# takah29/2d-fluid-simulator

Measured on AMD Instinct MI355X. Metric: simulation steps/sec + Poisson-sweep HBM GB/s (% roofline), res 4096², 1/2/4/8 GPU, higher is better.
Workload: dtype f32; 1 GPU; bc=5 res=4096 (8192x4096 cells) scheme=cip vc=5.0 RB-SOR(1.3, 2 iters) Re=1e+06 dt=0.05/res; BASELINE.json configs[2]; cells=33554432, fluid_cells=22424499, parallelism=y-slab x1

## Files before the change

### 2d-fluid-simulator_amd/csrc/fs_core.hip

```cpp
#include <algorithm>
#include <cstdio>
#include <cstdlib>
#include <cstring>
#include <cxxabi.h>
#include <mutex>
#include <numeric>
#include <type_traits>
#include <unordered_map>

#include "fs_launch.h"
#include "fs_tracer.h"

namespace fs {

static thread_local std::string g_err;
void set_error(const std::string &msg) { g_err = msg; }
int hip_fail(hipError_t e, const char *what, const char *file, int line)
{
    char buf[512];
    snprintf(buf, sizeof buf, "HIP error %d (%s) in %s at %s:%d", (int)e, hipGetErrorString(e), what, file, line);
    g_err = buf;
    return FS_ERR_HIP;
}

// ... 83 lines not shown
        c->prof_ms[r.name_id] += ms;
        c->prof_pool.push_back(r.start);
        c->prof_pool.push_back(r.stop);
    }
    c->prof_recs.clear();
    return FS_OK;
}

const fs_ctx::TileList *tile_list(fs_ctx *c, int lanes, int rt, bool stacked, int group, int nbx, int nby, int cls, int reach, int wgw, int jb, int je, int parent_rt)
{
    if (c->h_act4.empty() || nbx > 0xfff || nby > 0xffff || lanes > 4 || c->rows > 0xffff) return nullptr;
    if (je < 0) je = c->rows;
    if (parent_rt == rt) parent_rt = 0;
    if (parent_rt && (wgw != 1 || parent_rt % rt != 0 || parent_rt > 64)) return nullptr;
    if (cls == 3 && !(rt == 8 && parent_rt == 16 && wgw == 1 && lanes == 2)) return nullptr;
    const fs_ctx::TileKey key{{lanes, rt, stacked ? 1 : 0, group, cls, reach, wgw, parent_rt, jb, je}};
    auto it = c->tile_lists.find(key);
    if (it != c->tile_lists.end()) return it->second.d ? &it->second : nullptr;
    if (c->capturing || c->tape_rec || c->tile_lists.size() >= 512) { ++c->tile_list_misses; return nullptr; }
    const std::vector<uint8_t> &act = lanes == 4 ? c->h_act4 : (lanes == 2 ? c->h_act2 : c->h_act2w);
    const int ow = geo_owners(lanes), waves = (c->X / geo_cells(lanes) + ow - 1) / ow, Y = c->rows;
    std::vector<uint32_t> per[8];
    bool any_hint = false;
    auto plain_box = [&](int wx0, int wx1, int p0, int p1) -> bool {
        if (wx0 <= 0 || wx1 >= waves || p0 - reach < 0 || p1 + reach > Y) return false;
        for (int wx = wx0; wx < wx1; ++wx)
            for (int j = p0 - reach; j < p1 + reach; ++j)
                if (act[(size_t)wx * Y + j] & 2) return false;
        return true;
    };
    const int groups = (nby + group - 1) / group;
    constexpr bool col_major = true;
    for (int xcd = 0; xcd < 8; ++xcd)
        for (int lg = 0; lg * 8 + xcd < groups; ++lg)
            for (int o = 0; o < group * nbx; ++o) {
                const int ly = col_major ? o % group : o / nbx, bx = col_major ? o / group : o % nbx;
                const int by = (lg * 8 + xcd) * group + ly;
                if (by >= nby) continue;
                {
                    const int wx0 = stacked ? bx : bx * wgw, wx1 = std::min(waves, stacked ? bx + 1 : bx * wgw + wgw);
                    const int j0 = jb + (stacked ? by * wgw : by) * rt, j1 = std::min(je, jb + (stacked ? by * wgw + wgw : by + 1) * rt);
                    bool any = false;
                    for (int wx = wx0; wx < wx1 && !any; ++wx)
                        for (int j = j0; j < j1; ++j)
                            if (act[(size_t)wx * Y + j] & 1) { any = true; break; }
                    if (cls == 3) {
                        const int p0 = jb + (j0 - jb) / parent_rt * parent_rt, p1 = std::min(je, p0 + parent_rt);
                        if (p1 - p0 == parent_rt && plain_box(wx0, wx1, p0, p1)) {
                            if (j0 == p0) per[xcd].push_back((1u << 28) | ((uint32_t)by << 12) | (uint32_t)bx);
                        } else if (any) {
                            uint32_t h = 0u;
                            for (int s = 0; s < 2; ++s)
                                for (int j = j0 + 4 * s; j < std::min(j1, j0 + 4 * s + 4); ++j)
                                    if (act[(size_t)bx * Y + j] & 4) { h |= 2u << s; break; }
                            per[xcd].push_back((h << 28) | ((uint32_t)by << 12) | (uint32_t)bx);
                        }
                        any_hint = true;
                        continue;
                    }
                    if (any && cls) {
                        int p0 = j0, p1 = j1, full_rows = (stacked ? wgw : 1) * rt;
                        if (parent_rt) { p0 = jb + (j0 - jb) / parent_rt * parent_rt; p1 = std::min(je, p0 + parent_rt); full_rows = parent_rt; }
                        any = (p1 - p0 == full_rows && plain_box(wx0, wx1, p0, p1)) == (cls == 1);
                    }
                    uint32_t hints = 0u;
// ... 3 lines not shown
                            const int t0 = jb + (stacked ? by * wgw + w : by) * rt, t1 = std::min(je, t0 + rt);
                            if (wx >= waves || t0 >= je) continue;
                            const bool plain = plain_box(wx, wx + 1, t0, t1);
                            if (plain) hints |= 1u << w;
                        }
                        any_hint = any_hint || hints != 0u;
                    }
                    if (any && cls == 2 && wgw == 1) {
                        for (int j = j0; j < j1; ++j)
                            if (act[(size_t)bx * Y + j] & 4) { hints |= 2u; break; }
                    }
                    if (any) per[xcd].push_back((hints << 28) | ((uint32_t)by << 12) | (uint32_t)bx);
                }
            }
    if ((!cls || cls == 3) && any_hint && wgw == 1) {
        for (auto &v : per) std::stable_partition(v.begin(), v.end(), [](uint32_t e) { return ((e >> 28) & 1u) == 0u; });
    }
    size_t K = 0, total = 0;
    for (auto &v : per) total += v.size();
    if (total >= 64) {
        const size_t target = (total + 7) / 8;
        for (int d = 0; d < 8; ++d)
            while (per[d].size() > target) {
                int r = 0;
                for (int x = 1; x < 8; ++x) if (per[x].size() < per[r].size()) r = x;
                if (per[r].size() >= target) break;
                const size_t n = std::min(per[d].size() - target, target - per[r].size());
                per[r].insert(per[r].end(), per[d].end() - n, per[d].end());
                per[d].resize(per[d].size() - n);
            }
    }
    for (auto &v : per) K = std::max(K, v.size());
    fs_ctx::TileList tl;
    if (K > 0 && (cls || any_hint || total < (size_t)nbx * nby)) {
        std::vector<uint32_t> h(K * 8, 0xffffffffu);
        for (int xcd = 0; xcd < 8; ++xcd)
            for (size_t k = 0; k < per[xcd].size(); ++k) h[k * 8 + xcd] = per[xcd][k];
        if (hipMalloc(&tl.d, h.size() * sizeof(uint32_t)) == hipSuccess &&
            hipMemcpyAsync(tl.d, h.data(), h.size() * sizeof(uint32_t), hipMemcpyHostToDevice, c->stream) == hipSuccess &&
            hipStreamSynchronize(c->stream) == hipSuccess)
            { tl.per_xcd = (int)K; tl.count = (int)total; }
        else { if (tl.d) hipFree(tl.d); tl.d = nullptr; }
    }
    auto &slot = c->tile_lists[key] = tl;
    return slot.d ? &slot : nullptr;
}

static void tile_lists_free(fs_ctx *c)
{
    for (auto &kv : c->tile_lists) if (kv.second.d) hipFree(kv.second.d);
    c->tile_lists.clear();
}

int check_rows(const fs_ctx *c, int jb, int je)
{
    if (!(0 <= jb && jb <= je && je <= c->rows)) {
// ... 345 lines not shown
        int bv = 0, bd = 0;
        e = hipGetDeviceProperties(&prop, device);
        if (e == hipSuccess) e = dtype == 0 ? hipOccupancyMaxActiveBlocksPerMultiprocessor(&bv, k_velocity_bc_limit<float>, 256, 0)
                                            : hipOccupancyMaxActiveBlocksPerMultiprocessor(&bv, k_velocity_bc_limit<double>, 256, 0);
        if (e == hipSuccess) e = dtype == 0 ? hipOccupancyMaxActiveBlocksPerMultiprocessor(&bd, k_dye_bc_limit<float>, 256, 0)
                                            : hipOccupancyMaxActiveBlocksPerMultiprocessor(&bd, k_dye_bc_limit<double>, 256, 0);
        if (e == hipSuccess) c->barrier_wgs = std::min(bv, bd) * prop.multiProcessorCount / 2;
    }
    c->nwx = (nx / 4 + 61) / 62;
    if (e != hipSuccess) { fs_destroy(c); return hip_fail(e, "hipMalloc(ctx)", __FILE__, __LINE__); }
    if (const char *s = getenv("FS_MARCH")) c->use_march = atoi(s) != 0;
    if (const char *s = getenv("FS_TILE_LIST")) c->tile_list_mask = atoi(s);
    if (const char *s = getenv("FS_LIMIT_GATE")) c->limit_gate = atoi(s) != 0;
    if (const char *s = getenv("FS_FUSE_K2")) c->fuse_k2 = std::max(0, std::min(2, atoi(s)));
    if (const char *s = getenv("FS_RBPAIR_SPLIT")) c->rbpair_split = atoi(s);
    if (const char *s = getenv("FS_SMALL_CELLS")) c->small_cells = (size_t)atoll(s);
    c->stack_mask = XCD_RBSOR | XCD_ADVECT | XCD_GRAD;
    c->use_pairs = c->use_march && nx % 2 == 0;
    if (nx % 4 != 0) c->use_march = false;
    *out = c;
    return FS_OK;
}

int fs_destroy(fs_ctx *ctx)
{
    if (!ctx) return FS_OK;
    hipSetDevice(ctx->device);
    if (ctx->stream) hipStreamSynchronize(ctx->stream);
    fs_comm_destroy(ctx);
    for (auto g : ctx->graphs) if (g) hipGraphExecDestroy(g);
// ... 111 lines not shown
    tile_lists_free(ctx);
    ctx->h_act4.clear(); ctx->h_act2.clear(); ctx->h_act2w.clear();
    if (ctx->X % 2 == 0 && ctx->tile_list_mask && ctx->rows <= 0xffff) {
        const int X = ctx->X, Y = ctx->Y, R = ctx->rows, g0 = ctx->y0 - ctx->halo;
        struct Geo { std::vector<uint8_t> *act; int w, halo; } geos[3] = {{&ctx->h_act4, 248, 4}, {&ctx->h_act2, 120, 4}, {&ctx->h_act2w, 124, 2}};
        for (const Geo &ge : geos) {
            const int w = ge.w, n = (X + w - 1) / w;
            ge.act->assign((size_t)n * R, 0);
            for (int i = 0; i < X; ++i) {
                const uint8_t *m = mask_xy + (size_t)i * Y, *b = ctx->h_bcmap.data() + (size_t)i * Y;
                uint8_t *a = ge.act->data() + (size_t)(i / w) * R;
                const int r = i % w;
                uint8_t *h = r < ge.halo && i / w > 0 ? a - R : (r >= w - ge.halo && i / w + 1 < n ? a + R : nullptr);
                for (int lr = 0; lr < R; ++lr) {
                    const int j = g0 + lr;
                    if (j < 0 || j >= Y) { a[lr] |= 2; if (h) h[lr] |= 2; continue; }
                    const uint8_t nf = m[j] != 0 ? 2 : 4;
                    a[lr] |= (uint8_t)((m[j] != 1) | (b[j] != 0)) | nf;
                    if (h) h[lr] |= nf;
                }
            }
        }
    }
    std::vector<uint8_t>().swap(ctx->h_bcmap);
    if (rc) return rc;
    if (ctx->X % 4 == 0) {
        FS_KLAUNCH(k_lazy_flags, dim3((ctx->nwx * ctx->rows + 3) / 4), dim3(256), 0, ctx->stream, ctx->grid(), ctx->nwx, ctx->d_bcmap, ctx->d_lazyflags);
        FS_HIP(hipGetLastError());
        const size_t cap = (size_t)ctx->nwx * ctx->rows;
        if (!ctx->d_pairlist) FS_HIP(hipMalloc(&ctx->d_pairlist, (2 * cap + 2) * sizeof(uint32_t)));
        unsigned *d_count = (unsigned *)(ctx->d_pairlist + 2 * cap);
        FS_HIP(hipMemsetAsync(d_count, 0, 2 * sizeof(unsigned), ctx->stream));
// ... 1275 lines not shown
```

### 2d-fluid-simulator_amd/csrc/fs_host.h

```cpp
#pragma once
#include <hip/hip_runtime.h>
#include <stdint.h>

#include <array>
#include <cmath>
#include <functional>
#include <map>
#include <set>
#include <string>
#include <vector>

#include "../../include/fs_hip.h"
#include "fs_device.h"
#include "fs_kernels.h"
#include "fs_march.h"
#include "fs_rbpair.h"
#include "fs_jquad.h"
#include "fs_k34n.h"
#include "fs_history.h"

namespace fs {

void set_error(const std::string &msg);
int hip_fail(hipError_t e, const char *what, const char *file, int line);
// ... 44 lines not shown

struct fs_ctx {
    int device = 0;
    int X = 0, Y = 0, dtype = 0, y0 = 0, nyl = 0, halo = 0;
    int rows = 0, P = 0, Pm = 0;
    size_t esize = 4;
    hipStream_t stream = nullptr;
    uint8_t *d_mask = nullptr;
    uint8_t *d_bcmap = nullptr;
    uint8_t *d_lazyflags = nullptr;
    std::vector<uint8_t> h_bcmap;
    bool lazy_ok = false;
    bool rb_pair_ok = false;
    bool jq_ok = false;
    int rbpair_split = 1;
    size_t small_cells = (size_t)1 << 21;
    uint32_t *d_pairlist = nullptr; int n_pairlist[2] = {0, 0};
    int nwx = 0;
    void *d_bc_const = nullptr, *d_bc_dye = nullptr;
    bool mask_set = false, bc_incomplete = false;
    int bc_radius_vel = 0, bc_radius_prs = 0;
    fs::BcOpsDev ops_vel, ops_prs, ops_dye;
    void *d_stage = nullptr;
    size_t stage_bytes = 0;
    double *d_acc = nullptr;
    int barrier_wgs = 0;
    unsigned *d_sync = nullptr;
    double *d_partial = nullptr;
    size_t partial_cap = 0;
    double *d_stats = nullptr;
// ... 19 lines not shown
    std::set<fs_history *> histories;
    std::vector<fs_history *> deferred_hist;
    std::set<fs_mean *> means;
    std::vector<fs_mean *> deferred_mean;
    std::set<fs_tracer *> tracers;
    std::vector<fs_tracer *> deferred_tracer;
    std::vector<void *> deferred_accum;
    bool use_march = true;
    bool use_pairs = true;
    int fuse_k2 = 2;
    bool limit_gate = true;
    int stack_mask = 0;

    int tile_list_mask = 1 | 2 | 4 | 8 | 32;
    std::vector<uint8_t> h_act4, h_act2, h_act2w;
    struct TileList { uint32_t *d = nullptr; int per_xcd = 0; int count = 0; };
    using TileKey = std::array<int, 10>;
    std::map<TileKey, TileList> tile_lists;

    fs::Grid grid() const
    {
        fs::Grid g;
        g.tiles = nullptr;
        g.X = X; g.P = P; g.Pm = Pm; g.rows = rows;
        int jlo = halo - y0, jhi = halo - y0 + (Y - 1);
        g.jlo = jlo < 0 ? 0 : jlo;
        g.jhi = jhi > rows - 1 ? rows - 1 : jhi;
        g.ybase = y0 - halo;
        g.mask = d_mask;
        return g;
    }
};
// ... 109 lines not shown
```

### 2d-fluid-simulator_amd/csrc/fs_pressure.hip

```cpp
#include "fs_launch.h"
#include "fs_stats.h"
#include "fs_mean.h"

static_assert(fs::STATS_N == FS_FLOW_NSTAT, "fs_stats.h and include/fs_hip.h disagree on the slots");
static_assert(fs::MEAN_PLANES == FS_MEAN_NPLANE, "fs_mean.h and include/fs_hip.h disagree on the planes");

namespace fs {
void history_release(fs_history *h)
{
    if (h->d_probes) hipFree(h->d_probes);
    if (h->d_faces) hipFree(h->d_faces);
    if (h->d_ring) hipFree(h->d_ring);
    if (h->d_state) hipFree(h->d_state);
    if (h->d_partial) hipFree(h->d_partial);
    delete h;
}
void mean_release(fs_mean *m)
{
    if (m->d_sums) hipFree(m->d_sums);
    if (m->d_state) hipFree(m->d_state);
    delete m;
}
}

// ... 186 lines not shown
    FS_REQUIRE(pc_out != pc && pc_out != pn && pn != pc, "the finishing pass needs three distinct pressure fields");
    FS_ROWS();
    if (!(ctx->jq_ok && ctx->use_march && ctx->dtype == 0)) { set_error("this mask / precision does not admit the multi-sweep Jacobi passes (fs_jacobi_quad_ok)"); return FS_ERR_UNSUPPORTED; }
    using T = float;
    const OvGrid og = ov_grid_lanes(ctx, row_begin, row_end, 4, 1, XCD_RBSOR, 2, true, 0, 2);
    return launch(ctx, "jacobi_finish", [=] {
        FS_KLAUNCH((k_jacobi_finish<2, 4, T>), og.grid, dim3(og.threads), 0, ctx->stream, og.g, og.nbx, og.nby, row_begin, row_end,
                           (const uint8_t *)ctx->d_bcmap, (T *)pc_out->d, (T *)pn->d, (const T *)pc->d, (const T *)src->d);
    });
}

int fs_rbsor_pair_ok(const fs_ctx *ctx, int *ok)
{
    FS_REQUIRE(ctx && ok, "null argument");
    *ok = ctx->mask_set && ctx->rb_pair_ok && ctx->use_pairs ? 1 : 0;
    return FS_OK;
}

int fs_rbsor_pair(fs_ctx *ctx, double dt, double dx, double omega, fs_field *pc_out, fs_field *pn_out, const fs_field *pc, const fs_field *pn,
                  const fs_field *vc, int full, int row_begin, int row_end)
{
    FS_REQUIRE(ctx, "ctx is null");
    FS_FIELD(pc_out, 1); FS_FIELD(pn_out, 1); FS_FIELD(pc, 1); FS_FIELD(pn, 1); FS_FIELD(vc, 2);
    FS_REQUIRE(pc_out != pn_out && pc_out != pc && pc_out != pn && pn_out != pc && pn_out != pn && pc != pn, "the two-iteration pass needs four distinct pressure fields");
    FS_ROWS();
    if (!(ctx->rb_pair_ok && ctx->use_pairs)) {
        set_error("this mask does not admit the two-iteration red-black pass (fs_rbsor_pair_ok)");
        return FS_ERR_UNSUPPORTED;
    }
    const Grid gg = ctx->grid();
// ... 402 lines not shown
```

### 2d-fluid-simulator_amd/csrc/fs_rbpair.h

```cpp
#pragma once
#include "fs_march.h"

namespace fs {

#ifndef FS_RBP_MIRROR
#define FS_RBP_MIRROR 1
#endif

template <typename T, int N> struct LV { T a[N]; };
template <typename T, int N> struct LVec;
template <> struct LVec<float, 4> { using type = float4; };
template <> struct LVec<float, 2> { using type = float2; };
template <> struct LVec<double, 2> { using type = double2; };
template <int N> struct LMaskWord;
template <> struct LMaskWord<4> { using type = uint32_t; };
template <> struct LMaskWord<2> { using type = uint16_t; };

template <typename T, int N>
__device__ __forceinline__ LV<T, N> lv_load(const T *row, int i0)
{
    const typename LVec<T, N>::type q = load_row_quad<typename LVec<T, N>::type, T>(row, i0);
    LV<T, N> r;
    if constexpr (N == 4) { r.a[0] = q.x; r.a[1] = q.y; r.a[2] = q.z; r.a[3] = q.w; }
    else { r.a[0] = q.x; r.a[1] = q.y; }
// ... 165 lines not shown

template <typename T, int N>
__device__ __forceinline__ LV<T, N> lv_bc_row(const LaneMapN<N> &lm, const LV<T, N> &m, const LV<T, N> &c, const LV<T, N> &n, uint32_t code)
{
    if (!__any(lv_sel_target<N>(code) != 0u)) return c;
    const T cl = lv_left<T, N>(lm, c), cr = lv_right<T, N>(lm, c);
    LV<T, N> o;
#pragma unroll
    for (int q = 0; q < N; ++q) {
        const T sL = q == 0 ? cl : c.a[q == 0 ? 0 : q - 1], sR = q == N - 1 ? cr : c.a[q == N - 1 ? q : q + 1];
        o.a[q] = lazy_value((code >> (8 * q)) & 0xffu, c.a[q], sL, sR, m.a[q], n.a[q]);
    }
    return o;
}

template <int PAR, int COLOR, typename T, int N>
__device__ __forceinline__ void rbp_relax(const Konst<T> &k, const LaneMapN<N> &lm, unsigned fluid, const LV<T, N> &m, const LV<T, N> &ctr, const LV<T, N> &p,
                                          const LV<T, N> &s2, const LV<T, N> &s3, LV<T, N> &out)
{
    const T pl = lv_left<T, N>(lm, ctr), pr = lv_right<T, N>(lm, ctr);
#pragma unroll
    for (int c = 0; c < N; ++c) {
        if (((c + PAR) & 1) != COLOR) continue;
        const T pE = c == N - 1 ? pr : ctr.a[c == N - 1 ? c : c + 1], pW = c == 0 ? pl : ctr.a[c == 0 ? 0 : c - 1];
        const T pred = predict_from(pE, pW, p.a[c], m.a[c], s2.a[c], s3.a[c]);
        const T val = k.om1 * ctr.a[c] + k.om * pred;
        out.a[c] = (fluid & (1u << c)) ? val : out.a[c];
    }
}

template <int N, int RT, int PAR0, int DM, bool BND, bool FULL, typename T, bool MIRROR = false>
__device__ __forceinline__ void rbsor_pair_tile(const Grid &g, const Konst<T> &k, const LaneMapN<N> &lm_in, int i0, int j0, int je, const unsigned (&fl)[RT + 8],
                                                const uint8_t *bcmap, T *C, T *D, const T *A, const T *B, const T *v)
{
    static_assert(!(MIRROR && (BND || FULL)), "only plain tiles are mirrored");
    constexpr int W = RT + 8;
    constexpr int UP = MIRROR ? -1 : 1;
    constexpr int PARW = MIRROR ? PAR0 + 1 : PAR0;
#define FS_ROW(w) (MIRROR ? j0 + RT + 3 - (w) : j0 - 4 + (w))
    using R = LV<T, N>;
    constexpr unsigned ALL = (1u << N) - 1u;
    const LaneMapN<N> lm = BND ? lm_in : LaneMapN<N>{lm_in.i0, lm_in.owner, false, false};
// ... 55 lines not shown
    }
#pragma unroll
    for (int w = 4; w <= W - 5; ++w) {
        const int j = FS_ROW(w);
        if (j >= je) continue;
        const unsigned sel = FULL ? ALL : (FS_FL(w) | (BND ? lv_sel_target<N>(code[w]) : 0u));
        if (lm.owner && sel) {
            lv_store_sel<T, N>(C + idx<1, T>(g, 0, i0, j), P4[w], sel);
            lv_store_sel<T, N>(D + idx<1, T>(g, 0, i0, j), VB[w], sel);
        }
    }
#undef FS_FL
#undef FS_ROW
}

template <int N, int RT, int PAR0, int DM, bool MIRROR, typename T>
__device__ __forceinline__ void rbsor_pair_stack_tile(const Grid &g, const Konst<T> &k, const LaneMapN<N> &lm_in, int i0, int j0,
                                                      T *C, T *D, const T *A, const T *B, const T *v, typename LVec<T, N>::type (*xch)[2][64], int slot)
{
    constexpr int W = RT + 5;
    constexpr int UP = MIRROR ? -1 : 1;
    constexpr int PARW = MIRROR ? PAR0 + 1 : PAR0;
#define FS_ROW(w) (MIRROR ? j0 + RT + 3 - (w) : j0 - 4 + (w))
    using R = LV<T, N>;
    using Q = typename LVec<T, N>::type;
    constexpr unsigned ALL = (1u << N) - 1u;
    const LaneMapN<N> lm{lm_in.i0, lm_in.owner, false, false};
    const int lane = threadIdx.x & 63;
    R PA[W], VX[W], VY[W], PB[W];
#pragma unroll
    for (int w = 0; w < W; ++w) {
        const int j = clampy(g, FS_ROW(w));
        PA[w] = lv_field<1, T, N>(A, g, 0, i0, j);
// ... 3 lines not shown
    }
    R S2[W], S3[W];
#pragma unroll
    for (int w = 1; w <= W - 2; ++w) {
        const T xl = lv_left<T, N>(lm, VX[w]), xr = lv_right<T, N>(lm, VX[w]);
        const T yl = lv_left<T, N>(lm, VY[w]), yr = lv_right<T, N>(lm, VY[w]);
#pragma unroll
        for (int c = 0; c < N; ++c) {
            const T xE = c == N - 1 ? xr : VX[w].a[c == N - 1 ? c : c + 1], xW = c == 0 ? xl : VX[w].a[c == 0 ? 0 : c - 1];
            const T yE = c == N - 1 ? yr : VY[w].a[c == N - 1 ? c : c + 1], yW = c == 0 ? yl : VY[w].a[c == 0 ? 0 : c - 1];
            source_from<DM>(k, xE, xW, yE, yW, VX[w + UP].a[c], VX[w - UP].a[c], VY[w + UP].a[c], VY[w - UP].a[c], S2[w].a[c], S3[w].a[c]);
        }
    }
    auto put = [&](int e, const R &r) { Q q; q.x = r.a[0]; q.y = r.a[1]; xch[e][slot][lane] = q; };
    auto get = [&](int e) { const Q q = xch[e][1 - slot][lane]; R r; r.a[0] = q.x; r.a[1] = q.y; return r; };
#pragma unroll
    for (int w = 1; w <= W - 2; ++w) {
        if ((PARW + w) & 1) rbp_relax<1, 1>(k, lm, ALL, PA[w - UP], PA[w], PA[w + UP], S2[w], S3[w], PB[w]);
        else                rbp_relax<0, 1>(k, lm, ALL, PA[w - UP], PA[w], PA[w + UP], S2[w], S3[w], PB[w]);
    }
    put(0, PB[W - 2]);
    __syncthreads();
    PB[W - 1] = get(0);
    R P2[W];
#pragma unroll
    for (int w = 2; w <= W - 2; ++w) {
        P2[w] = PB[w];
        if ((PARW + w) & 1) rbp_relax<1, 0>(k, lm, ALL, PB[w - UP], PB[w], PB[w + UP], S2[w], S3[w], P2[w]);
        else                rbp_relax<0, 0>(k, lm, ALL, PB[w - UP], PB[w], PB[w + UP], S2[w], S3[w], P2[w]);
    }
    put(1, P2[W - 2]);
    __syncthreads();
    P2[W - 1] = get(1);
    R P3[W];
#pragma unroll
    for (int w = 3; w <= W - 2; ++w) {
        P3[w] = PA[w];
        if ((PARW + w) & 1) rbp_relax<1, 1>(k, lm, ALL, P2[w - UP], P2[w], P2[w + UP], S2[w], S3[w], P3[w]);
        else                rbp_relax<0, 1>(k, lm, ALL, P2[w - UP], P2[w], P2[w + UP], S2[w], S3[w], P3[w]);
    }
    put(2, P3[W - 2]);
    __syncthreads();
    P3[W - 1] = get(2);
    R P4[W];
#pragma unroll
    for (int w = 4; w <= W - 2; ++w) {
        P4[w] = P3[w];
        if ((PARW + w) & 1) rbp_relax<1, 0>(k, lm, ALL, P3[w - UP], P3[w], P3[w + UP], S2[w], S3[w], P4[w]);
        else                rbp_relax<0, 0>(k, lm, ALL, P3[w - UP], P3[w], P3[w + UP], S2[w], S3[w], P4[w]);
    }
    if (lm.owner) {
#pragma unroll
        for (int w = 4; w <= W - 2; ++w) {
            lv_store_row<1, T, N>(C, g, 0, i0, FS_ROW(w), P4[w]);
            lv_store_row<1, T, N>(D, g, 0, i0, FS_ROW(w), P2[w]);
        }
    }
#undef FS_ROW
}

template <int N, int RT, int PAR0, int DM, int PATH, bool FULL, typename T>
__device__ __forceinline__ void rbsor_pair_wave_at(const Grid &g, const Konst<T> &k, int wx, int ty, bool hint, bool bnd_fluid, int jb, int je,
                                                   const uint8_t *bcmap, T *C, T *D, const T *A, const T *B, const T *v)
{
    constexpr int W = RT + 8;
    const LaneMapN<N> lm = lane_map_n<N>(g, wx);
// ... 42 lines not shown

template <int N, int PAR0, int DM, typename T>
__global__ __launch_bounds__(128) void k_rbsor_pair_all(Grid g, Konst<T> k, int nbx, int nby, int jb, int je, const uint8_t *bcmap, T *C, T *D, const T *A, const T *B, const T *v)
{
    constexpr int RT = 8;
    __shared__ typename LVec<T, N>::type xch[3][2][64];
    constexpr int OW = 64 - 2 * (4 / N);
    int wx, ty, cg;
    unsigned cls = 0u;
    if (!band_coords<1>(g, nbx, nby, wx, ty, cg, 0, &cls)) return;
    if (!(wx * OW < g.X / N && jb + ty * RT < je)) return;
    const int w = __builtin_amdgcn_readfirstlane((int)(threadIdx.x >> 6));
    if (cls & 1u) {
        const LaneMapN<N> lm = lane_map_n<N>(g, wx);
        const int j0 = jb + ty * RT;
        if (w == 0) rbsor_pair_stack_tile<N, RT, PAR0, DM, false, T>(g, k, lm, lm.i0, j0, C, D, A, B, v, xch, 0);
        else        rbsor_pair_stack_tile<N, RT, PAR0, DM, true, T>(g, k, lm, lm.i0, j0 + RT, C, D, A, B, v, xch, 1);
    } else {
        const int t4 = ty * 2 + w;
        if (jb + t4 * 4 >= je) return;
        rbsor_pair_wave_at<N, 4, PAR0, DM, 2, false, T>(g, k, wx, t4, false, ((cls >> (1 + w)) & 1u) != 0u, jb, je, bcmap, C, D, A, B, v);
    }
}

template <int N, int RT, int PAR0, int DM, int PATH, bool FULL, typename T>
__global__ __launch_bounds__(256, (PATH == 3 && sizeof(T) == 4 ? 4 : 1)) void k_rbsor_pair(Grid g, Konst<T> k, int nbx, int nby, int jb, int je,
                                                    const uint8_t *bcmap, T *C, T *D, const T *A, const T *B, const T *v)
{
    static_assert(RT % 2 == 0, "the row parity of a tile is a launch constant only for even tile heights");
    rbsor_pair_wave<N, RT, PAR0, DM, PATH, FULL, T>(g, k, nbx, nby, jb, je, bcmap, C, D, A, B, v);
}

// ... 3 lines not shown
```

### 2d-fluid-simulator_amd/fs/_lib.py

```python
import ctypes
import os

_HERE = os.path.dirname(os.path.abspath(__file__))
LIB_PATH = os.environ.get("FS_LIB") or os.path.join(os.path.dirname(_HERE), "csrc", "libfs_hip.so")
ABI_VERSION = 15

_lib = None

_c_int, _c_dbl, _c_vp, _c_sz = ctypes.c_int, ctypes.c_double, ctypes.c_void_p, ctypes.c_size_t
_P = ctypes.POINTER

_ROWS = [_c_int, _c_int]
_PROTOS = {
    "fs_abi_version": [],
    "fs_device_count": [_P(_c_int)],
    "fs_tile_list_stats": [_c_vp, _P(_c_int), _P(_c_int)],
    "fs_create": [_P(_c_vp), _c_int, _c_int, _c_int, _c_int, _c_int, _c_int, _c_int],
    "fs_destroy": [_c_vp],
    "fs_sync": [_c_vp],
    "fs_ctx_info": [_c_vp] + [_P(_c_int)] * 7,
    "fs_upload_mask": [_c_vp, _c_vp],
    "fs_upload_bc_const": [_c_vp, _c_vp],
    "fs_upload_bc_dye": [_c_vp, _c_vp],
    "fs_bc_radius": [_c_vp, _P(_c_int), _P(_c_int)],
# ... 10 lines not shown
    "fs_velocity_bc_limit": [_c_vp, _c_dbl, _c_vp, _c_int, _c_int, _c_int] + _ROWS,
    "fs_dye_bc_limit_ok": [_c_vp, _P(_c_int)],
    "fs_dye_bc_limit": [_c_vp, _c_dbl, _c_vp, _c_vp, _c_int, _c_int] + _ROWS,
    "fs_pressure_bc": [_c_vp, _c_vp] + _ROWS,
    "fs_dye_bc": [_c_vp, _c_vp] + _ROWS,
    "fs_mac_update": [_c_vp, _c_int, _c_dbl, _c_dbl, _c_dbl, _c_vp, _c_vp, _c_vp] + _ROWS,
    "fs_mac_dye": [_c_vp, _c_int, _c_dbl, _c_dbl, _c_vp, _c_vp, _c_vp] + _ROWS,
    "fs_cip_set_grad": [_c_vp, _c_dbl, _c_vp, _c_vp, _c_vp] + _ROWS,
    "fs_cip_nonadv": [_c_vp, _c_dbl, _c_dbl, _c_dbl, _c_vp, _c_vp, _c_vp] + _ROWS,
    "fs_cip_nonadv_dye": [_c_vp, _c_dbl, _c_dbl, _c_dbl, _c_vp, _c_vp] + _ROWS,
    "fs_cip_nonadv_grad": [_c_vp, _c_dbl] + [_c_vp] * 6 + _ROWS,
    "fs_cip_advect": [_c_vp, _c_dbl, _c_dbl] + [_c_vp] * 7 + _ROWS,
    "fs_cip_grad_advect": [_c_vp, _c_dbl, _c_dbl] + [_c_vp] * 7 + [_c_int] + _ROWS,
    "fs_cip_step_ok": [_c_vp, _P(_c_int)],
    "fs_cip_step_tiles": [_c_vp] + [_P(_c_int)] * 5,
    "fs_cip_step": [_c_vp, _c_dbl, _c_dbl, _c_dbl] + [_c_vp] * 8 + [_c_int] + _ROWS,
    "fs_cip_step_dye": [_c_vp, _c_dbl, _c_dbl, _c_dbl] + [_c_vp] * 8 + [_c_int, _c_int] + _ROWS,
    "fs_cip_grad_advect_dye": [_c_vp, _c_dbl, _c_dbl] + [_c_vp] * 8 + [_c_int, _c_int] + _ROWS,
    "fs_vort_calc": [_c_vp, _c_dbl, _c_vp, _c_vp, _c_vp] + _ROWS,
    "fs_vort_add": [_c_vp, _c_dbl, _c_dbl, _c_dbl, _c_vp, _c_vp, _c_vp, _c_vp] + _ROWS,
    "fs_vort_confine": [_c_vp, _c_dbl, _c_dbl, _c_dbl, _c_vp, _c_vp, _c_vp, _c_vp] + _ROWS,
    "fs_jacobi_sweep": [_c_vp, _c_dbl, _c_dbl, _c_vp, _c_vp, _c_vp] + _ROWS,
    "fs_rbsor_halfsweep": [_c_vp, _c_dbl, _c_dbl, _c_dbl, _c_int, _c_vp, _c_vp, _c_vp] + _ROWS,
    "fs_rbsor_iteration": [_c_vp, _c_dbl, _c_dbl, _c_dbl, _c_vp, _c_vp, _c_vp] + _ROWS,
    "fs_poisson_source": [_c_vp, _c_dbl, _c_dbl, _c_vp, _c_vp] + _ROWS,
    "fs_jacobi_sweep_src": [_c_vp, _c_vp, _c_vp, _c_vp] + _ROWS,
    "fs_lazy_bc_ok": [_c_vp, _P(_c_int)],
    "fs_jacobi_sweep_lazy": [_c_vp, _c_vp, _c_vp, _c_vp] + _ROWS,
    "fs_jacobi_pair_lazy": [_c_vp, _c_vp, _c_vp, _c_vp, _c_int] + _ROWS,
    "fs_jacobi_quad_ok": [_c_vp, _P(_c_int)],
# ... 121 lines not shown
```

### 2d-fluid-simulator_amd/fs/runtime.py

```python
import ctypes
import itertools
import os
import time
import weakref

import numpy as np

from . import _lib

_DTYPES = {"f32": np.float32, "f64": np.float64, np.float32: np.float32, np.float64: np.float64,
           np.dtype("float32"): np.float32, np.dtype("float64"): np.float64}

_config = {
    "gpu": 0, "dtype": np.float32, "rank": 0, "nranks": 1, "halo": None,
    "bcast": None,
    "allgather": None,
    "device_cls": None,
}
_devices = []
_serials = itertools.count(1)


def init(gpu=0, dtype="f32", rank=0, nranks=1, halo=None, bcast=None, allgather=None, device_cls=None):
    if dtype not in _DTYPES:
# ... 1106 lines not shown
        return bool(ok.value)

    has_cip_step = True

    @property
    def cip_step_fused(self):
        ok = ctypes.c_int()
        _lib.call("fs_cip_step_ok", self._ctx, ctypes.byref(ok))
        return bool(ok.value)

    def cip_step_tiles(self):
        v = [ctypes.c_int() for _ in range(5)]
        _lib.call("fs_cip_step_tiles", self._ctx, *[ctypes.byref(x) for x in v])
        return tuple(x.value for x in v)

    @property
    def jacobi_quad_ok(self):
        ok = ctypes.c_int()
        _lib.call("fs_jacobi_quad_ok", self._ctx, ctypes.byref(ok))
        return bool(ok.value) and self.nranks == 1

    def _p_exchange(self, h, nchan, depth):
        _lib.call("fs_halo_exchange", self._ctx, h, depth)

    def _p_exchange_many(self, handles, depth):
        self._p_exchange_begin(handles, depth)
        self._p_exchange_wait()

    def _p_exchange_begin(self, handles, depth):
        arr = (ctypes.c_void_p * len(handles))(*[h for h, _, _ in handles])
# ... 294 lines not shown
```

### include/fs_hip.h

```cpp
#ifndef FS_HIP_H
#define FS_HIP_H

#include <stddef.h>
#include <stdint.h>

#ifdef __cplusplus
extern "C" {
#endif

#define FS_ABI_VERSION 15

typedef struct fs_ctx fs_ctx;
typedef struct fs_field fs_field;

enum fs_status {
    FS_OK = 0,
    FS_ERR_ARG = -1,
    FS_ERR_HIP = -2,
    FS_ERR_STATE = -3,
    FS_ERR_COMM = -4,
    FS_ERR_UNSUPPORTED = -5
};

enum fs_scheme { FS_UPWIND = 0, FS_KK = 1 };

// ... 74 lines not shown
                       fs_field *pn, const fs_field *pc, const fs_field *vc, int row_begin, int row_end);
int fs_rbsor_iteration(fs_ctx *ctx, double dt, double dx, double omega, fs_field *pn, const fs_field *pc,
                       const fs_field *vc, int row_begin, int row_end);
int fs_poisson_source(fs_ctx *ctx, double dt, double dx, fs_field *src, const fs_field *vc,
                      int row_begin, int row_end);
int fs_jacobi_sweep_src(fs_ctx *ctx, fs_field *pn, const fs_field *pc, const fs_field *src,
                        int row_begin, int row_end);
int fs_lazy_bc_ok(const fs_ctx *ctx, int *ok);
int fs_jacobi_sweep_lazy(fs_ctx *ctx, fs_field *pn, const fs_field *pc, const fs_field *src, int row_begin, int row_end);
int fs_lazy_flags(fs_ctx *ctx, uint8_t *out, int capacity, int *wave_columns, int *rows, int *general_rows);
int fs_jacobi_pair_lazy(fs_ctx *ctx, fs_field *pn, const fs_field *pc, const fs_field *src, int mode, int row_begin, int row_end);
int fs_selftest_f64div(fs_ctx *ctx, double divisor, int *mismatches);
int fs_rbsor_pair_ok(const fs_ctx *ctx, int *ok);
int fs_rbsor_pair(fs_ctx *ctx, double dt, double dx, double omega, fs_field *pc_out, fs_field *pn_out, const fs_field *pc,
                  const fs_field *pn, const fs_field *vc, int full, int row_begin, int row_end);
int fs_jacobi_quad_ok(const fs_ctx *ctx, int *ok);
int fs_jacobi_quad_lazy(fs_ctx *ctx, fs_field *pn, const fs_field *pc, const fs_field *src, int row_begin, int row_end);
int fs_jacobi_finish(fs_ctx *ctx, fs_field *pc_out, fs_field *pn, const fs_field *pc, const fs_field *src, int row_begin, int row_end);
int fs_rbsor_halfsweep_src(fs_ctx *ctx, double omega, int parity, fs_field *pn, const fs_field *pc,
                           const fs_field *src, int row_begin, int row_end);
int fs_poisson_residual(fs_ctx *ctx, double dt, double dx, const fs_field *p, const fs_field *vc,
                        double *sum_sq, double *count);

#define FS_FLOW_NSTAT 10
int fs_flow_stats(fs_ctx *ctx, double dx, const fs_field *v, const fs_field *p, const int *box, double *out);

typedef struct fs_history fs_history;
int fs_history_create(fs_ctx *ctx, int npoints, const int *points, int nfaces, const int *faces, int capacity, int every, fs_history **out);
int fs_history_record(fs_ctx *ctx, fs_history *h, double dx, double limit, const fs_field *v, const fs_field *p);
int fs_history_read(fs_ctx *ctx, fs_history *h, double *out, int max_records, int *n_records, long long *launches, int *dropped);
// ... 99 lines not shown
```

Measured before the change: 1834 steps/s.

## Add column-uniform tile class for fused RB-SOR pair kernel

Adds a third tile class to the RB-SOR pair tile list: parent tiles whose wave column has uniform mask and boundary codes along rows. These tiles run the fast stacked 16-row path with per-lane fluid masks and a per-column boundary-condition recipe, instead of the slower general 4-row path. New activity flag bits (8, 16) mark row-to-row changes and unsupported BC kinds, and tile ordering now sorts three ranks. It also exposes tile-kind counts through a new diagnostic API. The risk is extra per-cell select work in the fast path and correctness near obstacles.

```diff
diff --git a/2d-fluid-simulator_amd/csrc/fs_core.hip b/2d-fluid-simulator_amd/csrc/fs_core.hip
--- a/2d-fluid-simulator_amd/csrc/fs_core.hip
+++ b/2d-fluid-simulator_amd/csrc/fs_core.hip
@@ -121,7 +121,8 @@
     if (parent_rt == rt) parent_rt = 0;
     if (parent_rt && (wgw != 1 || parent_rt % rt != 0 || parent_rt > 64)) return nullptr;
     if (cls == 3 && !(rt == 8 && parent_rt == 16 && wgw == 1 && lanes == 2)) return nullptr;
-    const fs_ctx::TileKey key{{lanes, rt, stacked ? 1 : 0, group, cls, reach, wgw, parent_rt, jb, je}};
+    const bool colu = cls == 3 && c->rbpair_colu != 0;
+    const fs_ctx::TileKey key{{lanes, rt, stacked ? 1 : 0, group, cls, reach, wgw, parent_rt, jb, je, colu ? 1 : 0}};
     auto it = c->tile_lists.find(key);
     if (it != c->tile_lists.end()) return it->second.d ? &it->second : nullptr;
     if (c->capturing || c->tape_rec || c->tile_lists.size() >= 512) { ++c->tile_list_misses; return nullptr; }
@@ -136,6 +137,13 @@
                 if (act[(size_t)wx * Y + j] & 2) return false;
         return true;
     };
+    auto column_uniform = [&](int wx, int p0, int p1) -> bool {
+        if (wx <= 0 || wx >= waves - 1 || (wx + 1) * ow * geo_cells(lanes) + 4 > c->X || p0 - reach < 0 || p1 + reach > Y) return false;
+        for (int j = p0 - reach; j < p1 + reach; ++j)
+            if ((act[(size_t)wx * Y + j] & 16) || (j > p0 - reach && (act[(size_t)wx * Y + j] & 8))) return false;
+        return true;
+    };
+    int kinds[3] = {0, 0, 0};
     const int groups = (nby + group - 1) / group;
     constexpr bool col_major = true;
     for (int xcd = 0; xcd < 8; ++xcd)
@@ -153,9 +161,14 @@
                             if (act[(size_t)wx * Y + j] & 1) { any = true; break; }
                     if (cls == 3) {
                         const int p0 = jb + (j0 - jb) / parent_rt * parent_rt, p1 = std::min(je, p0 + parent_rt);
+                        bool parent_work = false;
+                        for (int j = p0; j < p1 && !parent_work; ++j) parent_work = (act[(size_t)bx * Y + j] & 1) != 0;
                         if (p1 - p0 == parent_rt && plain_box(wx0, wx1, p0, p1)) {
-                            if (j0 == p0) per[xcd].push_back((1u << 28) | ((uint32_t)by << 12) | (uint32_t)bx);
+                            if (j0 == p0) { per[xcd].push_back((1u << 28) | ((uint32_t)by << 12) | (uint32_t)bx); ++kinds[0]; }
+                        } else if (colu && p1 - p0 == parent_rt && parent_work && column_uniform(bx, p0, p1)) {
+                            if (j0 == p0) { per[xcd].push_back((8u << 28) | ((uint32_t)by << 12) | (uint32_t)bx); ++kinds[1]; }
                         } else if (any) {
+                            ++kinds[2];
                             uint32_t h = 0u;
                             for (int s = 0; s < 2; ++s)
                                 for (int j = j0 + 4 * s; j < std::min(j1, j0 + 4 * s + 4); ++j)
@@ -189,7 +202,8 @@
                 }
             }
     if ((!cls || cls == 3) && any_hint && wgw == 1) {
-        for (auto &v : per) std::stable_partition(v.begin(), v.end(), [](uint32_t e) { return ((e >> 28) & 1u) == 0u; });
+        auto rank = [](uint32_t e) { return (e >> 28) & 1u ? 2 : ((e >> 31) & 1u ? 1 : 0); };
+        for (auto &v : per) std::stable_sort(v.begin(), v.end(), [&](uint32_t a, uint32_t b) { return rank(a) < rank(b); });
     }
     size_t K = 0, total = 0;
     for (auto &v : per) total += v.size();
@@ -214,7 +228,7 @@
         if (hipMalloc(&tl.d, h.size() * sizeof(uint32_t)) == hipSuccess &&
             hipMemcpyAsync(tl.d, h.data(), h.size() * sizeof(uint32_t), hipMemcpyHostToDevice, c->stream) == hipSuccess &&
             hipStreamSynchronize(c->stream) == hipSuccess)
-            { tl.per_xcd = (int)K; tl.count = (int)total; }
+            { tl.per_xcd = (int)K; tl.count = (int)total; for (int q = 0; q < 3; ++q) tl.kinds[q] = kinds[q]; }
         else { if (tl.d) hipFree(tl.d); tl.d = nullptr; }
     }
     auto &slot = c->tile_lists[key] = tl;
@@ -590,6 +604,7 @@
     if (const char *s = getenv("FS_LIMIT_GATE")) c->limit_gate = atoi(s) != 0;
     if (const char *s = getenv("FS_FUSE_K2")) c->fuse_k2 = std::max(0, std::min(2, atoi(s)));
     if (const char *s = getenv("FS_RBPAIR_SPLIT")) c->rbpair_split = atoi(s);
+    if (const char *s = getenv("FS_RBPAIR_COLU")) c->rbpair_colu = atoi(s);
     if (const char *s = getenv("FS_SMALL_CELLS")) c->small_cells = (size_t)atoll(s);
     c->stack_mask = XCD_RBSOR | XCD_ADVECT | XCD_GRAD;
     c->use_pairs = c->use_march && nx % 2 == 0;
@@ -731,8 +746,10 @@
                 uint8_t *h = r < ge.halo && i / w > 0 ? a - R : (r >= w - ge.halo && i / w + 1 < n ? a + R : nullptr);
                 for (int lr = 0; lr < R; ++lr) {
                     const int j = g0 + lr;
-                    if (j < 0 || j >= Y) { a[lr] |= 2; if (h) h[lr] |= 2; continue; }
-                    const uint8_t nf = m[j] != 0 ? 2 : 4;
+                    if (j < 0 || j >= Y) { a[lr] |= 2 | 16; if (h) h[lr] |= 2 | 16; continue; }
+                    uint8_t nf = m[j] != 0 ? 2 : 4;
+                    if (j == 0 || lr == 0 || m[j] != m[j - 1] || ((b[j] ^ b[j - 1]) & 0x7f)) nf |= 8;
+                    if ((b[j] & 1) && (((b[j] >> 1) & 3) == 1 || (((b[j] >> 1) & 3) == 0 && ((b[j] >> 3) & 3) >= 2))) nf |= 16;
                     a[lr] |= (uint8_t)((m[j] != 1) | (b[j] != 0)) | nf;
                     if (h) h[lr] |= nf;
                 }
diff --git a/2d-fluid-simulator_amd/csrc/fs_host.h b/2d-fluid-simulator_amd/csrc/fs_host.h
--- a/2d-fluid-simulator_amd/csrc/fs_host.h
+++ b/2d-fluid-simulator_amd/csrc/fs_host.h
@@ -82,6 +82,7 @@
     bool rb_pair_ok = false;
     bool jq_ok = false;
     int rbpair_split = 1;
+    int rbpair_colu = 1;
     size_t small_cells = (size_t)1 << 21;
     uint32_t *d_pairlist = nullptr; int n_pairlist[2] = {0, 0};
     int nwx = 0;
@@ -131,8 +132,8 @@
 
     int tile_list_mask = 1 | 2 | 4 | 8 | 32;
     std::vector<uint8_t> h_act4, h_act2, h_act2w;
-    struct TileList { uint32_t *d = nullptr; int per_xcd = 0; int count = 0; };
-    using TileKey = std::array<int, 10>;
+    struct TileList { uint32_t *d = nullptr; int per_xcd = 0; int count = 0; int kinds[3] = {0, 0, 0}; };
+    using TileKey = std::array<int, 11>;
     std::map<TileKey, TileList> tile_lists;
 
     fs::Grid grid() const
diff --git a/2d-fluid-simulator_amd/csrc/fs_pressure.hip b/2d-fluid-simulator_amd/csrc/fs_pressure.hip
--- a/2d-fluid-simulator_amd/csrc/fs_pressure.hip
+++ b/2d-fluid-simulator_amd/csrc/fs_pressure.hip
@@ -224,6 +224,20 @@
 {
     FS_REQUIRE(ctx && ok, "null argument");
     *ok = ctx->mask_set && ctx->rb_pair_ok && ctx->use_pairs ? 1 : 0;
+    return FS_OK;
+}
+
+int fs_rbsor_pair_tiles(fs_ctx *ctx, int *plain_parents, int *column_uniform_parents, int *general_units)
+{
+    FS_REQUIRE(ctx && plain_parents && column_uniform_parents && general_units, "null argument");
+    *plain_parents = *column_uniform_parents = *general_units = 0;
+    if (!(ctx->mask_set && ctx->rb_pair_ok && ctx->use_pairs && ctx->dtype == 0) || ctx->capturing || ctx->tape_rec) return FS_OK;
+    if (!(ctx->rbpair_split == 2 || (ctx->rbpair_split == 1 && (size_t)ctx->X * ctx->Y >= ((size_t)1 << 20)))) return FS_OK;
+    const OvGrid og = ov_grid_lanes(ctx, 0, ctx->rows, 8, 1, XCD_RBSOR, 2, true, 3, 4, 1, 16, ctx->halo != 0);
+    for (const auto &kv : ctx->tile_lists)
+        if (kv.second.d && kv.second.d == og.g.tiles) {
+            *plain_parents = kv.second.kinds[0]; *column_uniform_parents = kv.second.kinds[1]; *general_units = kv.second.kinds[2];
+        }
     return FS_OK;
 }
 
diff --git a/2d-fluid-simulator_amd/csrc/fs_rbpair.h b/2d-fluid-simulator_amd/csrc/fs_rbpair.h
--- a/2d-fluid-simulator_amd/csrc/fs_rbpair.h
+++ b/2d-fluid-simulator_amd/csrc/fs_rbpair.h
@@ -203,7 +203,33 @@
     return o;
 }
 
-template <int PAR, int COLOR, typename T, int N>
+template <int N> struct RowRecipe { unsigned left, right, zero; };
+template <int N> __device__ __forceinline__ RowRecipe<N> row_recipe(uint32_t code)
+{
+    RowRecipe<N> r{0u, 0u, 0u};
+#pragma unroll
+    for (int q = 0; q < N; ++q) {
+        const unsigned b = (code >> (8 * q)) & 0xffu, kind = (b >> 1) & 3u, d1 = (b >> 3) & 3u;
+        if ((b & 1u) && kind == 2u) r.zero |= 1u << q;
+        else if ((b & 1u) && d1 == 1u) r.right |= 1u << q;
+        else if (b & 1u) r.left |= 1u << q;
+    }
+    return r;
+}
+template <typename T, int N>
+__device__ __forceinline__ LV<T, N> lv_bc_row_own(const LV<T, N> &c, const RowRecipe<N> &rr)
+{
+    const T cl = lane_prev(c.a[N - 1]), cr = lane_next(c.a[0]);
+    LV<T, N> o;
+#pragma unroll
+    for (int q = 0; q < N; ++q) {
+        const T sL = q == 0 ? cl : c.a[q == 0 ? 0 : q - 1], sR = q == N - 1 ? cr : c.a[q == N - 1 ? q : q + 1];
+        o.a[q] = (rr.left & (1u << q)) ? sL : ((rr.right & (1u << q)) ? sR : ((rr.zero & (1u << q)) ? (T)0.0 : c.a[q]));
+    }
+    return o;
+}
+
+template <int PAR, int COLOR, bool BITSEL = false, typename T, int N>
 __device__ __forceinline__ void rbp_relax(const Konst<T> &k, const LaneMapN<N> &lm, unsigned fluid, const LV<T, N> &m, const LV<T, N> &ctr, const LV<T, N> &p,
                                           const LV<T, N> &s2, const LV<T, N> &s3, LV<T, N> &out)
 {
@@ -214,7 +240,10 @@
         const T pE = c == N - 1 ? pr : ctr.a[c == N - 1 ? c : c + 1], pW = c == 0 ? pl : ctr.a[c == 0 ? 0 : c - 1];
         const T pred = predict_from(pE, pW, p.a[c], m.a[c], s2.a[c], s3.a[c]);
         const T val = k.om1 * ctr.a[c] + k.om * pred;
-        out.a[c] = (fluid & (1u << c)) ? val : out.a[c];
+        if constexpr (BITSEL && sizeof(T) == 4) {
+            const unsigned mk = (fluid & (1u << c)) ? 0xffffffffu : 0u;
+            out.a[c] = __uint_as_float((__float_as_uint(val) & mk) | (__float_as_uint(out.a[c]) & ~mk));
+        } else out.a[c] = (fluid & (1u << c)) ? val : out.a[c];
     }
 }
 
@@ -300,9 +329,10 @@
 #undef FS_ROW
 }
 
-template <int N, int RT, int PAR0, int DM, bool MIRROR, typename T>
+template <int N, int RT, int PAR0, int DM, bool MIRROR, bool COLU, typename T>
 __device__ __forceinline__ void rbsor_pair_stack_tile(const Grid &g, const Konst<T> &k, const LaneMapN<N> &lm_in, int i0, int j0,
-                                                      T *C, T *D, const T *A, const T *B, const T *v, typename LVec<T, N>::type (*xch)[2][64], int slot)
+                                                      T *C, T *D, const T *A, const T *B, const T *v, typename LVec<T, N>::type (*xch)[2][64], int slot,
+                                                      unsigned fluid = (1u << N) - 1u, const RowRecipe<N> &rr = RowRecipe<N>{0u, 0u, 0u})
 {
     constexpr int W = RT + 5;
     constexpr int UP = MIRROR ? -1 : 1;
@@ -336,10 +366,14 @@
     }
     auto put = [&](int e, const R &r) { Q q; q.x = r.a[0]; q.y = r.a[1]; xch[e][slot][lane] = q; };
     auto get = [&](int e) { const Q q = xch[e][1 - slot][lane]; R r; r.a[0] = q.x; r.a[1] = q.y; return r; };
+    const unsigned FL = COLU ? fluid : ALL;
+    R VA[W];
+#pragma unroll
+    for (int w = 0; w < W; ++w) VA[w] = COLU ? lv_bc_row_own<T, N>(PA[w], rr) : PA[w];
 #pragma unroll
     for (int w = 1; w <= W - 2; ++w) {
-        if ((PARW + w) & 1) rbp_relax<1, 1>(k, lm, ALL, PA[w - UP], PA[w], PA[w + UP], S2[w], S3[w], PB[w]);
-        else                rbp_relax<0, 1>(k, lm, ALL, PA[w - UP], PA[w], PA[w + UP], S2[w], S3[w], PB[w]);
+        if ((PARW + w) & 1) rbp_relax<1, 1, COLU>(k, lm, FL, VA[w - UP], VA[w], VA[w + UP], S2[w], S3[w], PB[w]);
+        else                rbp_relax<0, 1, COLU>(k, lm, FL, VA[w - UP], VA[w], VA[w + UP], S2[w], S3[w], PB[w]);
     }
     put(0, PB[W - 2]);
     __syncthreads();
@@ -348,18 +382,22 @@
 #pragma unroll
     for (int w = 2; w <= W - 2; ++w) {
         P2[w] = PB[w];
-        if ((PARW + w) & 1) rbp_relax<1, 0>(k, lm, ALL, PB[w - UP], PB[w], PB[w + UP], S2[w], S3[w], P2[w]);
-        else                rbp_relax<0, 0>(k, lm, ALL, PB[w - UP], PB[w], PB[w + UP], S2[w], S3[w], P2[w]);
+        if ((PARW + w) & 1) rbp_relax<1, 0, COLU>(k, lm, FL, PB[w - UP], PB[w], PB[w + UP], S2[w], S3[w], P2[w]);
+        else                rbp_relax<0, 0, COLU>(k, lm, FL, PB[w - UP], PB[w], PB[w + UP], S2[w], S3[w], P2[w]);
     }
     put(1, P2[W - 2]);
     __syncthreads();
     P2[W - 1] = get(1);
+    if constexpr (COLU) {
+#pragma unroll
+        for (int w = 2; w <= W - 1; ++w) P2[w] = lv_bc_row_own<T, N>(P2[w], rr);
+    }
     R P3[W];
 #pragma unroll
     for (int w = 3; w <= W - 2; ++w) {
-        P3[w] = PA[w];
-        if ((PARW + w) & 1) rbp_relax<1, 1>(k, lm, ALL, P2[w - UP], P2[w], P2[w + UP], S2[w], S3[w], P3[w]);
-        else                rbp_relax<0, 1>(k, lm, ALL, P2[w - UP], P2[w], P2[w + UP], S2[w], S3[w], P3[w]);
+        P3[w] = VA[w];
+        if ((PARW + w) & 1) rbp_relax<1, 1, COLU>(k, lm, FL, P2[w - UP], P2[w], P2[w + UP], S2[w], S3[w], P3[w]);
+        else                rbp_relax<0, 1, COLU>(k, lm, FL, P2[w - UP], P2[w], P2[w + UP], S2[w], S3[w], P3[w]);
     }
     put(2, P3[W - 2]);
     __syncthreads();
@@ -368,10 +406,19 @@
 #pragma unroll
     for (int w = 4; w <= W - 2; ++w) {
         P4[w] = P3[w];
-        if ((PARW + w) & 1) rbp_relax<1, 0>(k, lm, ALL, P3[w - UP], P3[w], P3[w + UP], S2[w], S3[w], P4[w]);
-        else                rbp_relax<0, 0>(k, lm, ALL, P3[w - UP], P3[w], P3[w + UP], S2[w], S3[w], P4[w]);
-    }
-    if (lm.owner) {
+        if ((PARW + w) & 1) rbp_relax<1, 0, COLU>(k, lm, FL, P3[w - UP], P3[w], P3[w + UP], S2[w], S3[w], P4[w]);
+        else                rbp_relax<0, 0, COLU>(k, lm, FL, P3[w - UP], P3[w], P3[w + UP], S2[w], S3[w], P4[w]);
+    }
+    if constexpr (COLU) {
+        const unsigned sel = fluid | rr.left | rr.right | rr.zero;
+        if (lm.owner && sel) {
+#pragma unroll
+            for (int w = 4; w <= W - 2; ++w) {
+                lv_store_row_sel<1, T, N>(C, g, 0, i0, FS_ROW(w), P4[w], sel);
+                lv_store_row_sel<1, T, N>(D, g, 0, i0, FS_ROW(w), P2[w], sel);
+            }
+        }
+    } else if (lm.owner) {
 #pragma unroll
         for (int w = 4; w <= W - 2; ++w) {
             lv_store_row<1, T, N>(C, g, 0, i0, FS_ROW(w), P4[w]);
@@ -444,8 +491,15 @@
     if (cls & 1u) {
         const LaneMapN<N> lm = lane_map_n<N>(g, wx);
         const int j0 = jb + ty * RT;
-        if (w == 0) rbsor_pair_stack_tile<N, RT, PAR0, DM, false, T>(g, k, lm, lm.i0, j0, C, D, A, B, v, xch, 0);
-        else        rbsor_pair_stack_tile<N, RT, PAR0, DM, true, T>(g, k, lm, lm.i0, j0 + RT, C, D, A, B, v, xch, 1);
+        if (w == 0) rbsor_pair_stack_tile<N, RT, PAR0, DM, false, false, T>(g, k, lm, lm.i0, j0, C, D, A, B, v, xch, 0);
+        else        rbsor_pair_stack_tile<N, RT, PAR0, DM, true, false, T>(g, k, lm, lm.i0, j0 + RT, C, D, A, B, v, xch, 1);
+    } else if (cls & 8u) {
+        const LaneMapN<N> lm = lane_map_n<N>(g, wx);
+        const int j0 = jb + ty * RT;
+        const unsigned fluid = lv_sel_fluid<N>(lv_bytes<N>(g.mask, g, lm.i0, j0));
+        const RowRecipe<N> rr = row_recipe<N>(lv_bytes<N>(bcmap, g, lm.i0, j0));
+        if (w == 0) rbsor_pair_stack_tile<N, RT, PAR0, DM, false, true, T>(g, k, lm, lm.i0, j0, C, D, A, B, v, xch, 0, fluid, rr);
+        else        rbsor_pair_stack_tile<N, RT, PAR0, DM, true, true, T>(g, k, lm, lm.i0, j0 + RT, C, D, A, B, v, xch, 1, fluid, rr);
     } else {
         const int t4 = ty * 2 + w;
         if (jb + t4 * 4 >= je) return;
diff --git a/2d-fluid-simulator_amd/fs/_lib.py b/2d-fluid-simulator_amd/fs/_lib.py
--- a/2d-fluid-simulator_amd/fs/_lib.py
+++ b/2d-fluid-simulator_amd/fs/_lib.py
@@ -3,7 +3,7 @@
 
 _HERE = os.path.dirname(os.path.abspath(__file__))
 LIB_PATH = os.environ.get("FS_LIB") or os.path.join(os.path.dirname(_HERE), "csrc", "libfs_hip.so")
-ABI_VERSION = 15
+ABI_VERSION = 16
 
 _lib = None
 
@@ -48,6 +48,7 @@
     "fs_cip_grad_advect": [_c_vp, _c_dbl, _c_dbl] + [_c_vp] * 7 + [_c_int] + _ROWS,
     "fs_cip_step_ok": [_c_vp, _P(_c_int)],
     "fs_cip_step_tiles": [_c_vp] + [_P(_c_int)] * 5,
+    "fs_rbsor_pair_tiles": [_c_vp] + [_P(_c_int)] * 3,
     "fs_cip_step": [_c_vp, _c_dbl, _c_dbl, _c_dbl] + [_c_vp] * 8 + [_c_int] + _ROWS,
     "fs_cip_step_dye": [_c_vp, _c_dbl, _c_dbl, _c_dbl] + [_c_vp] * 8 + [_c_int, _c_int] + _ROWS,
     "fs_cip_grad_advect_dye": [_c_vp, _c_dbl, _c_dbl] + [_c_vp] * 8 + [_c_int, _c_int] + _ROWS,
diff --git a/2d-fluid-simulator_amd/fs/runtime.py b/2d-fluid-simulator_amd/fs/runtime.py
--- a/2d-fluid-simulator_amd/fs/runtime.py
+++ b/2d-fluid-simulator_amd/fs/runtime.py
@@ -1144,6 +1144,11 @@
         _lib.call("fs_cip_step_tiles", self._ctx, *[ctypes.byref(x) for x in v])
         return tuple(x.value for x in v)
 
+    def rbsor_pair_tiles(self):
+        v = [ctypes.c_int() for _ in range(3)]
+        _lib.call("fs_rbsor_pair_tiles", self._ctx, *[ctypes.byref(x) for x in v])
+        return tuple(x.value for x in v)
+
     @property
     def jacobi_quad_ok(self):
         ok = ctypes.c_int()
diff --git a/include/fs_hip.h b/include/fs_hip.h
--- a/include/fs_hip.h
+++ b/include/fs_hip.h
@@ -8,7 +8,7 @@
 extern "C" {
 #endif
 
-#define FS_ABI_VERSION 15
+#define FS_ABI_VERSION 16
 
 typedef struct fs_ctx fs_ctx;
 typedef struct fs_field fs_field;
@@ -113,6 +113,7 @@
 int fs_rbsor_pair_ok(const fs_ctx *ctx, int *ok);
 int fs_rbsor_pair(fs_ctx *ctx, double dt, double dx, double omega, fs_field *pc_out, fs_field *pn_out, const fs_field *pc,
                   const fs_field *pn, const fs_field *vc, int full, int row_begin, int row_end);
+int fs_rbsor_pair_tiles(fs_ctx *ctx, int *plain_parents, int *column_uniform_parents, int *general_units);
 int fs_jacobi_quad_ok(const fs_ctx *ctx, int *ok);
 int fs_jacobi_quad_lazy(fs_ctx *ctx, fs_field *pn, const fs_field *pc, const fs_field *src, int row_begin, int row_end);
 int fs_jacobi_finish(fs_ctx *ctx, fs_field *pc_out, fs_field *pn, const fs_field *pc, const fs_field *src, int row_begin, int row_end);
```

Measured after the change: 1846 steps/s, median of 6. About the same (+0.6%).
